# telin0411/multimodal_sequencing

Hardware: AMD Instinct MI355X
Metric: multimodal steps/sec (fwd+bwd) at N=5 steps, seq=512, ViT-B/16; 1/2/4/8 GPU (higher is better)
Workload: dtype bf16; 1 GPU; config3: ViT-B/16 + 12x768 joint encoder + BERSON, N=5 steps, 20 pairs/story, pair seq 120+393=513; global_batch=32, stories_per_gpu=32, micro_batch=32, seq_len=513, parallelism=dp1

## Files before the change

multimodal_sequencing_amd/_native.py:

```python
import ctypes
import math
import os
import re

import torch

_HERE = os.path.dirname(os.path.abspath(__file__))
LIB_PATH = os.path.join(_HERE, "_lib", "libmmseq.so")
HEADER_PATH = os.path.join(os.path.dirname(_HERE), "include", "mmseq.h")

_vp = ctypes.c_void_p


class Rows(ctypes.Structure):
    _fields_ = [("ld", ctypes.c_int64), ("bstride", ctypes.c_int64), ("rpb", ctypes.c_int64)]


def rows(ld, bstride=0, rpb=1 << 62):
    return Rows(ld, bstride, rpb)


class Dropout(ctypes.Structure):
    _fields_ = [("p", ctypes.c_float), ("stream", ctypes.c_uint32), ("seed", ctypes.c_uint64)]

# ... 52 lines not shown
               for body, name in take(r"typedef\s+struct\s*\{([^}]*)\}\s*(\w+)\s*;")}
    sigs = {}
    for decl in filter(None, (d.strip() for d in text.split(";"))):
        if decl == "}":
            continue
        m = re.fullmatch(r"(mmseq_status|int64_t|const\s+char\s*\*)\s*(mmseq_\w+)\s*\(([^()]*)\)", decl)
        if not m:
            raise NativeError(f"mmseq.h: cannot parse declaration {' '.join(decl.split())!r}")
        args = [] if m[3].strip() in ("", "void") else m[3].split(",")
        sigs[m[2]] = (_RETURNS[re.sub(r"\s*\*", "*", " ".join(m[1].split()))],
                      [(_dp if re.search(r"\bmmseq_dropout\b", a) else _vp) if "*" in a
                       else scalar(a, m[2]) for a in args])
    return sigs, consts, structs


def _read_header():
    if not os.path.exists(HEADER_PATH):
        raise NativeError(f"mmseq C header not found at {HEADER_PATH}; the binding reads every "
                          "signature and constant from it.")
    with open(HEADER_PATH) as f:
        return f.read()


_SIGS, CONSTANTS, STRUCTS = parse_header(_read_header())

F32, BF16 = CONSTANTS["MMSEQ_F32"], CONSTANTS["MMSEQ_BF16"]
ACT = {"none": CONSTANTS["MMSEQ_ACT_NONE"], "gelu": CONSTANTS["MMSEQ_ACT_GELU_ERF"],
       "quickgelu": CONSTANTS["MMSEQ_ACT_QUICKGELU"], "tanh": CONSTANTS["MMSEQ_ACT_TANH"],
       "gelu_tanh": CONSTANTS["MMSEQ_ACT_GELU_TANH"]}
EUNSUPPORTED = CONSTANTS["MMSEQ_EUNSUPPORTED"]
XENT_EVAL_MAX_K = CONSTANTS["MMSEQ_XENT_EVAL_MAX_K"]

WORKSPACE_BYTES = 256 << 20
_ws = {}


def gemm_workspace(device, stream=None):
    dev = torch.device(device)
    if stream is None:
        stream = torch.cuda.current_stream(dev)
    key = (dev.index if dev.index is not None else torch.cuda.current_device(), stream.cuda_stream)
    buf = _ws.get(key)
    if buf is None:
        buf = _ws[key] = torch.empty(WORKSPACE_BYTES // 4, dtype=torch.float32, device=dev)
    return buf


GEMM_AUTO = CONSTANTS["MMSEQ_GEMM_AUTO"]
_sel = {"gemm": GEMM_AUTO, "attn": 1}
_lib = None


def lib():
    global _lib
    if _lib is None:
        if not os.path.exists(LIB_PATH):
            raise NativeError(
                f"mmseq HIP library not found at {LIB_PATH}; run __graft_entry__.build() "
                "(make -C multimodal_sequencing_amd/csrc). There is no CPU fallback.")
        L = ctypes.CDLL(LIB_PATH)
        for name, (res, args) in _SIGS.items():
            fn = getattr(L, name)
            fn.restype = res
            fn.argtypes = args
        _lib = L
    return _lib


def _check(st, what):
    if st != 0:
        raise NativeError(f"{what} failed ({st}): {lib().mmseq_last_error().decode()}")


def _status(st, name):
    if st != EUNSUPPORTED:
        _check(st, name)
# ... 123 lines not shown


def attn_fwd_rows(P, T, Tq, heads, qkv, key_bias, scale, out, lse, drop=None, keep_bits=None):
    _dev(qkv, out, lse)
    H = heads * 64
    _call("mmseq_attn_fwd_rows", P, T, Tq, heads, _p(qkv), 3 * H, 0, H, 2 * H, _p(key_bias), scale,
          _p(out), H, _p(lse), _d(drop), _p(keep_bits))


def attn_bwd_rows(P, T, Tq, heads, qkv, key_bias, scale, out, dout, lse, delta, dqkv, drop=None,
                  keep_bits=None):
    _dev(qkv, out, dout, dqkv)
    H = heads * 64
    _call("mmseq_attn_bwd_rows", P, T, Tq, heads, _p(qkv), 3 * H, 0, H, 2 * H, _p(key_bias), scale,
          _p(out), H, _p(dout), H, _p(lse), _p(delta), _p(dqkv), 3 * H, _d(drop), _p(keep_bits))


def small_attn_fwd(B, T, heads, d, q, k, v, key_bias, scale, out, probs, drop=None):
    _call("mmseq_small_attn_fwd", B, T, heads, d, _p(q), _p(k), _p(v), _p(key_bias), scale, _p(out),
          _p(probs), _d(drop))


def small_attn_bwd(B, T, heads, d, q, k, v, probs, dout, scale, dq, dk, dv, drop=None):
    _call("mmseq_small_attn_bwd", B, T, heads, d, _p(q), _p(k), _p(v), _p(probs), _p(dout), scale,
          _p(dq), _p(dk), _p(dv), _d(drop))


def layernorm_fwd(nrows, cols, x, xl, gamma, beta, eps, y, yl, mean, rstd, drop=None):
    _dev(x, y, gamma, beta)
    _call("mmseq_layernorm_fwd", nrows, cols, _p(x), xl, _p(gamma), _p(beta), eps, _p(y), yl,
# ... 626 lines not shown
```

multimodal_sequencing_amd/csrc/attention.hip:

```cpp
#include "gemm_common.h"
#include "launch_plan.h"
#include <type_traits>

namespace {

using namespace mmseq_plan;

constexpr int HD = 64;
constexpr int QT = 64;
constexpr float NEG = -1e30f;

template <typename TI> struct ACfg;
template <> struct ACfg<unsigned short> { static constexpr int LD = 80, VE = 8; };
template <> struct ACfg<float> { static constexpr int LD = 68, VE = 4; };

template <typename TI> struct V16;
template <> struct V16<unsigned short> { typedef u16x8 T; };
template <> struct V16<float> { typedef f32x4 T; };

struct AttnArgs {
  int P, T, heads;
  const void* qkv; int64_t ld_qkv, q_off, k_off, v_off;
  const float* key_bias; float scale;
  const void* out; int64_t ld_out;
  const void* dout; int64_t ld_dout;
  float* lse; float* delta;
  void* dqkv; int64_t ld_dqkv;
  void* o_w;
  Drop drop;
  uint64_t* bits;
  int nkt2;
  int tail0, nxq, xoff, nxl;
  int Tq;
  uint8_t* q8; int64_t ldq8; uint8_t* q8s;
};

template <typename TI>
__device__ __forceinline__ void stage_tile(TI* s, const TI* base, int64_t ld, int r0, int T,
                                           int tid) {
  typedef typename V16<TI>::T V;
  constexpr int VE = ACfg<TI>::VE, LD = ACfg<TI>::LD;
  constexpr int CPR = HD / VE;
  constexpr int NCH = (QT * CPR) / 256;
#pragma unroll
  for (int c = 0; c < NCH; ++c) {
    int L = c * 256 + tid;
    int r = L / CPR, cc = L % CPR;
    V v;
    if (r0 + r < T) {
// ... 1333 lines not shown
      unsigned short* op = reinterpret_cast<unsigned short*>(a.o_w) + ((int64_t)p * T + q) * a.ld_out +
                           h * 64 + 4 * hh;
#pragma unroll
      for (int db = 0; db < 2; ++db)
#pragma unroll
        for (int jj = 0; jj < 4; ++jj) {
          const f32x4 v = {o[qb][db][4 * jj], o[qb][db][4 * jj + 1], o[qb][db][4 * jj + 2],
                           o[qb][db][4 * jj + 3]};
          Vec4<unsigned short>::st(op + db * 32 + 8 * jj, v * inv);
        }
      if (hh == 0) a.lse[((int64_t)p * a.heads + h) * T + q] = (m[qb] + __builtin_amdgcn_logf(lt)) * LN2;
    }
  }
}

template <int DMODE>
__global__ __launch_bounds__(256, DMODE == 0 ? 4 : 2) void attn_dq_bf16_kernel(AttnArgs a) {
  constexpr bool DROP = DMODE != 0;
  extern __shared__ __attribute__((aligned(16))) unsigned short smem[];
  float* sBias = reinterpret_cast<float*>(smem + 4 * IMG);
  const int tid = threadIdx.x, lane = tid & 63;
  const int wave = __builtin_amdgcn_readfirstlane(tid >> 6);
  const int g = lane >> 4, i = lane & 15;
  const int T = a.T;
  const BlkIdx bi = attn_block((a.Tq + 127) >> 7, a.heads);
  const int h = bi.h, p = bi.p;
  const int nkt = (T + 63) >> 6;
  const int qw = bi.x * 128 + wave * 32;
  const bool active = qw < a.Tq;
  const int64_t ld = a.ld_qkv;
  const rsrc_t rk = head_rsrc(a.qkv, (int64_t)p * T, ld, a.k_off + h * 64, T);
  const rsrc_t rv = head_rsrc(a.qkv, (int64_t)p * T, ld, a.v_off + h * 64, T);
  const uint32_t loff = dma_lane_off(lane, ld);
  const rsrc_t rbits = DMODE == 2 ? make_rsrc(a.bits + ((int64_t)p * a.heads + h) * T * a.nkt2,
                                              (int64_t)T * a.nkt2 * 8)
                                  : make_rsrc(a.qkv, 0);
  const uint32_t boff0 = (uint32_t)(((qw + i) * a.nkt2 * 4 + g) * 2);
  auto stage = [&](int t) {
    unsigned short* kimg = smem + (t & 1) * 2 * IMG;
#pragma unroll
// ... 41 lines not shown
    for (int ks = 0; ks < 2; ++ks) {
      const u16x8 x = __builtin_bit_cast(u16x8, of[grp][ks]), y = __builtin_bit_cast(u16x8, ovf[grp][ks]);
#pragma unroll
      for (int e = 0; e < 8; ++e) dot = fmaf(bf2f(x[e]), bf2f(y[e]), dot);
    }
    dot += __shfl_xor(dot, 16, 64);
    dot += __shfl_xor(dot, 32, 64);
    Dd[grp] = dot;
    const int64_t ri = ((int64_t)p * a.heads + h) * T + q;
    L2[grp] = q < a.Tq ? L2[grp] * LOG2E : 1e30f;
    if (q < a.Tq && g == 0) a.delta[ri] = dot;
    settle(qf[grp][0]);
    settle(qf[grp][1]);
    settle(L2[grp]);
  }
  const float c = a.scale * LOG2E;
  const int Tp4 = (T + 3) & ~3;
  uint64_t drow[2];
#pragma unroll
  for (int grp = 0; grp < 2; ++grp)
    drow[grp] = (((uint64_t)p * a.heads + h) * T + (qw + grp * 16 + i)) * Tp4;
  constexpr bool DQ_LINIT = DMODE == 2;
  f32x4 linit[2];
#pragma unroll
  for (int grp = 0; grp < 2; ++grp) {
    const float nl = -L2[grp] / c;
    linit[grp] = (f32x4){nl, nl, nl, nl};
  }
  f32x4 dq[2][4];
#pragma unroll
// ... 73 lines not shown
      }
      dsf[grp][0] = pack_pair(dp[grp][0], dp[grp][1]);
      dsf[grp][1] = pack_pair(dp[grp][2], dp[grp][3]);
    }
#pragma unroll
    for (int d = 0; d < 4; ++d) {
      const bf16x8_t k0 = lds_tr(kimg, to[d]), k1 = lds_tr(kimg, 32 * 64 + to[d]);
#pragma unroll
      for (int grp = 0; grp < 2; ++grp) {
        dq[grp][d] = mma(k0, dsf[grp][0], dq[grp][d]);
        dq[grp][d] = mma(k1, dsf[grp][1], dq[grp][d]);
      }
    }
  }
  asm volatile("s_waitcnt vmcnt(0)" ::: "memory");
  if (!active) return;
#pragma unroll
  for (int grp = 0; grp < 2; ++grp) {
    const int q = qw + grp * 16 + i;
    if (q < T) {
      unsigned short* dqp = reinterpret_cast<unsigned short*>(a.dqkv) +
                            ((int64_t)p * T + q) * a.ld_dqkv + a.q_off + h * 64 + 4 * g;
#pragma unroll
      for (int d = 0; d < 4; ++d) Vec4<unsigned short>::st(dqp + d * 16, dq[grp][d] * a.scale);
      if (a.q8) q8_head_row(a, (int64_t)p * T + q, (int)a.q_off + h * 64, dq[grp], a.scale, g);
    }
  }
}

__device__ __forceinline__ void zero_dq(const AttnArgs& a, unsigned short* row, int h, int g) {
  unsigned short* dqp = row + a.q_off + h * 64 + 4 * g;
#pragma unroll
  for (int d = 0; d < 4; ++d) Vec4<unsigned short>::st(dqp + d * 16, (f32x4){0.f, 0.f, 0.f, 0.f});
}

template <int DMODE, bool FOLD>
__global__ __launch_bounds__(256, FOLD || DMODE == 1 ? 2 : 3) void attn_dkdv_bf16_kernel(AttnArgs a) {
  constexpr bool DROP = DMODE != 0;
  extern __shared__ __attribute__((aligned(16))) unsigned short smem[];
  const int T = a.T, Tq = a.Tq;
  const int nqt = (Tq + 63) >> 6;
  float* sL = reinterpret_cast<float*>(smem + 4 * IMG);
  float* sD = sL + nqt * 64;
  unsigned short* sBits = reinterpret_cast<unsigned short*>(sD + nqt * 64);
  unsigned short* sBitsT = sBits + 1024;
  u16x8* sKVt = reinterpret_cast<u16x8*>(sBitsT + 1024);
  const int tid = threadIdx.x, lane = tid & 63;
  const int wave = __builtin_amdgcn_readfirstlane(tid >> 6);
  const int g = lane >> 4, i = lane & 15;
  BlkIdx bi = attn_block(a.nxl, a.heads);
  bi.x += a.xoff;
// ... 271 lines not shown
        unsigned short* dkp = row + a.k_off + h * 64 + 4 * g;
        unsigned short* dvp = row + a.v_off + h * 64 + 4 * g;
#pragma unroll
        for (int d = 0; d < 4; ++d) {
          Vec4<unsigned short>::st(dkp + d * 16, dkt[d] * a.scale);
          Vec4<unsigned short>::st(dvp + d * 16, dvt[d]);
        }
        if (a.q8) {
          q8_head_row(a, (int64_t)p * T + key, (int)a.k_off + h * 64, dkt, a.scale, g);
          q8_head_row(a, (int64_t)p * T + key, (int)a.v_off + h * 64, dvt, 1.f, g);
        }
        if (key >= Tq) zero_dq(a, row, h, g);
      }
    }
  }
  if (!active) return;
#pragma unroll
  for (int grp = 0; grp < 2; ++grp) {
    const int key = kw + grp * 16 + i;
    if (key < T) {
      unsigned short* row = reinterpret_cast<unsigned short*>(a.dqkv) + ((int64_t)p * T + key) * a.ld_dqkv;
      unsigned short* dkp = row + a.k_off + h * 64 + 4 * g;
      unsigned short* dvp = row + a.v_off + h * 64 + 4 * g;
#pragma unroll
      for (int d = 0; d < 4; ++d) {
        Vec4<unsigned short>::st(dkp + d * 16, dk[grp][d] * a.scale);
        Vec4<unsigned short>::st(dvp + d * 16, dv[grp][d]);
      }
      if (a.q8) {
        q8_head_row(a, (int64_t)p * T + key, (int)a.k_off + h * 64, dk[grp], a.scale, g);
        q8_head_row(a, (int64_t)p * T + key, (int)a.v_off + h * 64, dv[grp], 1.f, g);
      }
      if (key >= Tq) zero_dq(a, row, h, g);
    }
  }
}

bool aligned16(const void* p) { return ((uintptr_t)p & 15) == 0; }

mmseq_status check_common(int P, int T, int heads, const void* qkv, int64_t ld, int64_t qo,
                          int64_t ko, int64_t vo, mmseq_dtype dt) {
  MMSEQ_REQUIRE(P >= 0 && T > 0 && heads > 0, "attn: bad sizes P=%d T=%d heads=%d", P, T, heads);
  MMSEQ_REQUIRE(dt == MMSEQ_F32 || dt == MMSEQ_BF16, "attn: bad dtype");
  const int ve = dt == MMSEQ_BF16 ? 8 : 4;
  MMSEQ_REQUIRE(aligned16(qkv) && ld % ve == 0 && qo % ve == 0 && ko % ve == 0 && vo % ve == 0,
                "attn: qkv must be 16-byte aligned with ld/offsets multiple of %d", ve);
  MMSEQ_REQUIRE(qo + heads * 64 <= ld && ko + heads * 64 <= ld && vo + heads * 64 <= ld,
                "attn: head slices exceed the row");
  return MMSEQ_OK;
// ... 14 lines not shown
typedef void (*AttnKernel)(AttnArgs);
typedef const AttnKernel FwdFamily[3][2];
FwdFamily FWD32 = {{attn_fwd32_kernel<0, false>, attn_fwd32_kernel<0, false>},
                   {attn_fwd32_kernel<1, false>, attn_fwd32_kernel<1, true>},
                   {attn_fwd32_kernel<2, false>, attn_fwd32_kernel<2, true>}};
FwdFamily FWD16 = {{attn_fwd_bf16_kernel<0, false>, attn_fwd_bf16_kernel<0, false>},
                   {attn_fwd_bf16_kernel<1, false>, attn_fwd_bf16_kernel<1, true>},
                   {attn_fwd_bf16_kernel<2, false>, attn_fwd_bf16_kernel<2, true>}};
FwdFamily FWD16_Q8 = {{attn_fwd_bf16_kernel<0, false, true>, attn_fwd_bf16_kernel<0, false, true>},
                      {attn_fwd_bf16_kernel<1, false, true>, attn_fwd_bf16_kernel<1, true, true>},
                      {attn_fwd_bf16_kernel<2, false, true>, attn_fwd_bf16_kernel<2, true, true>}};
const AttnKernel DQ16[3] = {attn_dq_bf16_kernel<0>, attn_dq_bf16_kernel<1>, attn_dq_bf16_kernel<2>};
const AttnKernel DKDV16[3][2] = {{attn_dkdv_bf16_kernel<0, false>, attn_dkdv_bf16_kernel<0, true>},
                                 {attn_dkdv_bf16_kernel<1, false>, nullptr},
                                 {attn_dkdv_bf16_kernel<2, false>, attn_dkdv_bf16_kernel<2, true>}};

void launch_fwd(FwdFamily& k, const AttnFwdPlan& p, const AttnArgs& a, hipStream_t s) {
  hipLaunchKernelGGL(k[p.dmode][p.wide], dim3(p.blocks), dim3(p.threads), (size_t)p.lds_bytes, s, a);
}

}

static mmseq_status attn_fwd_impl(int P, int T, int Tq, int heads, const void* qkv, int64_t ld_qkv,
                                  int64_t q_off, int64_t k_off, int64_t v_off,
                                  const float* key_bias, float scale, void* out, int64_t ld_out,
                                  float* lse, mmseq_dtype dtype, const mmseq_dropout* drop,
                                  uint64_t* keep_bits, int variant, mmseq_stream stream) {
  mmseq_status st = check_common(P, T, heads, qkv, ld_qkv, q_off, k_off, v_off, dtype);
  if (st) return st;
  MMSEQ_REQUIRE(out && lse && ld_out >= heads * 64, "attn_fwd: bad out/lse");
// ... 30 lines not shown
                                            int64_t v_off, const float* key_bias, float scale,
                                            void* out, int64_t ld_out, float* lse,
                                            const mmseq_dropout* drop, uint64_t* keep_bits,
                                            mmseq_stream stream) {
  return attn_fwd_impl(P, T, Tq, heads, qkv, ld_qkv, q_off, k_off, v_off, key_bias, scale, out,
                       ld_out, lse, MMSEQ_BF16, drop, keep_bits, 1, stream);
}

static mmseq_status attn_bwd_impl(int P, int T, int Tq, int heads, const void* qkv, int64_t ld_qkv,
                                  int64_t q_off, int64_t k_off, int64_t v_off,
                                  const float* key_bias, float scale, const void* out,
                                  int64_t ld_out, const void* dout, int64_t ld_dout,
                                  const float* lse, float* delta, void* dqkv, int64_t ld_dqkv,
                                  mmseq_dtype dtype, const mmseq_dropout* drop,
                                  const uint64_t* keep_bits, int variant, void* q8, int64_t ldq8,
                                  void* q8_scales, mmseq_stream stream) {
  mmseq_status st = check_common(P, T, heads, qkv, ld_qkv, q_off, k_off, v_off, dtype);
  if (st) return st;
  const int ve = dtype == MMSEQ_BF16 ? 8 : 4;
  MMSEQ_REQUIRE(out && dout && lse && delta && dqkv, "attn_bwd: null buffer");
  MMSEQ_REQUIRE(aligned16(dout) && ld_dout % ve == 0, "attn_bwd: dout alignment");
  const int64_t hi_off = q_off > k_off ? (q_off > v_off ? q_off : v_off) : (k_off > v_off ? k_off : v_off);
  MMSEQ_REQUIRE(hi_off + (int64_t)heads * 64 <= ld_dqkv,
                "attn_bwd: head slices exceed the dqkv row (ld_dqkv=%lld)", (long long)ld_dqkv);
  MMSEQ_REQUIRE(Tq >= 1 && Tq <= T && (Tq == T || (dtype == MMSEQ_BF16 && variant && !q8)),
                "attn_bwd: Tq=%d (1 <= Tq <= T; Tq < T needs the bf16 fast kernels, no MX-fp8 copy)", Tq);
  if (P == 0) return MMSEQ_OK;
  AttnArgs a = attn_args(P, T, Tq, heads, qkv, ld_qkv, q_off, k_off, v_off, key_bias, scale, drop, keep_bits);
  a.out = out; a.ld_out = ld_out; a.dout = dout; a.ld_dout = ld_dout;
  a.lse = const_cast<float*>(lse); a.delta = delta; a.dqkv = dqkv; a.ld_dqkv = ld_dqkv;
  a.q8 = reinterpret_cast<uint8_t*>(q8); a.ldq8 = ldq8; a.q8s = reinterpret_cast<uint8_t*>(q8_scales);
  if (q8 && !(dtype == MMSEQ_BF16 && variant))
    return mmseq_set_error(MMSEQ_EUNSUPPORTED, "attn_bwd_mxfp8: the bf16 fast kernels only");
  hipStream_t s = reinterpret_cast<hipStream_t>(stream);
  const int64_t rows = (int64_t)P * T;
  dim3 gd((unsigned)((rows + 3) / 4));
  dim3 grid((T + QT - 1) / QT, heads, P);
  if (dtype == MMSEQ_BF16 && variant) {
    MMSEQ_REQUIRE(aligned16(out) && ld_out % 8 == 0 && aligned16(dqkv) && ld_dqkv % 8 == 0,
                  "attn_bwd: out / dqkv must be 16-byte aligned rows");
    const AttnBwdPlan bp = attn_bwd_plan(P, T, Tq, heads, a.drop.thr != 0, keep_bits != nullptr);
    hipLaunchKernelGGL(DQ16[bp.dmode], dim3(bp.dq_blocks), dim3(256), (size_t)bp.dq_lds, s, a);
    AttnArgs ak = a;
    ak.tail0 = bp.tail0; ak.nxq = bp.nxq;
    ak.xoff = 0; ak.nxl = bp.nplain;
    if (bp.nplain)
      hipLaunchKernelGGL(DKDV16[bp.dmode][0], dim3(bp.plain_blocks), dim3(256), (size_t)bp.dkdv_lds, s, ak);
    ak.xoff = bp.nplain; ak.nxl = 1;
    if (bp.ntail)
      hipLaunchKernelGGL(DKDV16[bp.dmode][1], dim3(bp.tail_blocks), dim3(256), (size_t)bp.tail_lds, s, ak);
  } else if (dtype == MMSEQ_BF16) {
    hipLaunchKernelGGL(attn_delta_kernel<unsigned short>, gd, dim3(256), 0, s, a);
    hipLaunchKernelGGL(attn_dkdv_kernel<unsigned short>, grid, dim3(256), 0, s, a);
    hipLaunchKernelGGL(attn_dq_kernel<unsigned short>, grid, dim3(256), 0, s, a);
  } else {
// ... 2 lines not shown
    hipLaunchKernelGGL(attn_dq_kernel<float>, grid, dim3(256), 0, s, a);
  }
  return mmseq_check_launch("attn_bwd");
}

extern "C" mmseq_status mmseq_attn_bwd(int P, int T, int heads, const void* qkv, int64_t ld_qkv,
                                       int64_t q_off, int64_t k_off, int64_t v_off,
                                       const float* key_bias, float scale, const void* out,
                                       int64_t ld_out, const void* dout, int64_t ld_dout,
                                       const float* lse, float* delta, void* dqkv,
                                       int64_t ld_dqkv, mmseq_dtype dtype,
                                       const mmseq_dropout* drop, const uint64_t* keep_bits,
                                       int variant, mmseq_stream stream) {
  return attn_bwd_impl(P, T, T, heads, qkv, ld_qkv, q_off, k_off, v_off, key_bias, scale, out, ld_out,
                       dout, ld_dout, lse, delta, dqkv, ld_dqkv, dtype, drop, keep_bits, variant,
                       nullptr, 0, nullptr, stream);
}

extern "C" mmseq_status mmseq_attn_bwd_rows(int P, int T, int Tq, int heads, const void* qkv,
                                            int64_t ld_qkv, int64_t q_off, int64_t k_off,
                                            int64_t v_off, const float* key_bias, float scale,
                                            const void* out, int64_t ld_out, const void* dout,
                                            int64_t ld_dout, const float* lse, float* delta,
                                            void* dqkv, int64_t ld_dqkv, const mmseq_dropout* drop,
                                            const uint64_t* keep_bits, mmseq_stream stream) {
  return attn_bwd_impl(P, T, Tq, heads, qkv, ld_qkv, q_off, k_off, v_off, key_bias, scale, out, ld_out,
                       dout, ld_dout, lse, delta, dqkv, ld_dqkv, MMSEQ_BF16, drop, keep_bits, 1,
                       nullptr, 0, nullptr, stream);
}

extern "C" mmseq_status mmseq_attn_bwd_mxfp8(int P, int T, int heads, const void* qkv,
                                             int64_t ld_qkv, const float* key_bias, float scale,
                                             const void* out, int64_t ld_out, const void* dout,
                                             int64_t ld_dout, const float* lse, float* delta,
                                             void* dqkv, int64_t ld_dqkv,
                                             const mmseq_dropout* drop, const uint64_t* keep_bits,
                                             void* q8, int64_t ldq8, void* q8_scales,
                                             mmseq_stream stream) {
  const int64_t H = (int64_t)heads * 64;
  MMSEQ_REQUIRE(q8 && q8_scales && ldq8 >= 3 * H && ldq8 % 16 == 0 && ((uintptr_t)q8 & 15) == 0,
                "attn_bwd_mxfp8: q8 / ldq8");
  return attn_bwd_impl(P, T, T, heads, qkv, ld_qkv, 0, H, 2 * H, key_bias, scale, out, ld_out, dout,
                       ld_dout, lse, delta, dqkv, ld_dqkv, MMSEQ_BF16, drop, keep_bits, 1, q8, ldq8,
                       q8_scales, stream);
}

extern "C" int64_t mmseq_attn_keep_bits_words(int P, int T, int heads) {
  return keep_bits_words(P, T, heads);
}

extern "C" mmseq_status mmseq_attn_fwd_mxfp8_dual(int P, int T, int heads, const void* qkv,
                                                  int64_t ld_qkv, int64_t q_off, int64_t k_off,
                                                  int64_t v_off, const float* key_bias, float scale,
                                                  void* out, int64_t ld_out, float* lse,
                                                  const mmseq_dropout* drop, uint64_t* keep_bits,
                                                  void* q8, int64_t ldq8, void* q8_scales,
                                                  mmseq_stream stream) {
  mmseq_status st = check_common(P, T, heads, qkv, ld_qkv, q_off, k_off, v_off, MMSEQ_BF16);
  if (st) return st;
// ... 23 lines not shown
```

multimodal_sequencing_amd/csrc/launch_plan.h:

```cpp
#pragma once
#include <cstdint>

namespace mmseq_plan {

inline int64_t ceil_div(int64_t a, int64_t b) { return (a + b - 1) / b; }

constexpr int RCH = 64;

inline int reduce_rows(int nb) { return (int)ceil_div(nb, RCH); }
inline int64_t reduce_extra(int nb, int W) { return (int64_t)reduce_rows(nb) * W; }
inline int64_t partials_floats(int nb, int W) { return (int64_t)nb * W + reduce_extra(nb, W); }

constexpr int CS_ROWS = 256;

struct ColsumPlan {
  int nb;
  int64_t red_off;
  int64_t floats;
};

inline ColsumPlan colsum_plan(int rows, int cols) {
  const int nb = (int)ceil_div(rows, CS_ROWS);
  return {nb, (int64_t)nb * cols, partials_floats(nb, cols)};
}
// ... 142 lines not shown
  p.dmode = dropout ? (keep_bits ? 2 : 1) : 0;
  p.nkt2 = attn_nkt2(T);
  p.dq_blocks = attn_blocks((Tq + 127) / 128, heads, P);
  p.dq_lds = ATTN_KV_LDS + (int64_t)attn_nkt(T) * 64 * 4;
  const TailFold f = tail_fold(T, p.dmode != 1);
  p.tail0 = f.tail0; p.nxq = f.nxq;
  p.ntail = f.tail0 ? 1 : 0;
  p.nplain = f.nxq - p.ntail;
  p.plain_blocks = attn_blocks(p.nplain, heads, P);
  p.tail_blocks = attn_blocks(p.ntail, heads, P);
  p.dkdv_lds = ATTN_KV_LDS + (int64_t)attn_nkt(T) * 64 * 4 * 2 + 2048;
  p.tail_lds = p.dkdv_lds + 6144;
  return p;
}

}
```

multimodal_sequencing_amd/kernels.py:

```python
import math
import os

import torch

from . import _native as N

GELU, QGELU, TANH, GELU_TANH = (N.ACT[a] for a in ("gelu", "quickgelu", "tanh", "gelu_tanh"))


def _rows(ld):
    return N.rows(ld)


def _colsum(x, out):
    rows = x.numel() // x.shape[-1]
    N.colsum(x, rows, x.shape[-1], x.shape[-1], out, accumulate=True)


def _wgrad(dy, x, gW, gb=None):
    N.gemm_wgrad(dy, x, gW, gb)


def _linear(x, W, bias=None, act=0, aux=None, resid=None, out=None, out_dtype=None, drop=None):
    R = x.numel() // x.shape[-1]
# ... 154 lines not shown
                                                 dx_drop=dx_drop, drop_dx=drop_dx)), dsum
        N.layernorm_bwd(R, C, dy, _rows(C), x, _rows(C), mean, rstd, gamma, dx,
                        dx_rows if dx_rows is not None else _rows(C), dres, _rows(C), dgamma, dbeta,
                        dx_drop=dx_drop, drop_dx=drop_dx,
                        dx_drop_rows=dx_drop_rows, dsum=dsum, dsum_with_dres=dsum_with_dres)
        return _Act(g), None

    def attn_bwd(self, P, T, heads, qkv, key_bias, o, do, lse, drop=None, keep_bits=None, Tq=None):
        H = qkv.shape[-1] // 3
        scale = 1.0 / math.sqrt(H // heads)
        dqkv = torch.empty_like(qkv)
        delta = torch.empty(P, heads, T, device=qkv.device)
        if self.f8dg:
            return _Act(dqkv, N.attn_bwd_mxfp8(P, T, heads, qkv, key_bias, scale, o, do, lse, delta, dqkv,
                                               drop=drop, keep_bits=keep_bits))
        if Tq is not None and Tq < T:
            N.attn_bwd_rows(P, T, Tq, heads, qkv, key_bias, scale, o, do, lse, delta, dqkv, drop=drop,
                            keep_bits=keep_bits)
        else:
            N.attn_bwd(P, T, heads, qkv, 3 * H, 0, H, 2 * H, key_bias, scale, o, H, do, H, lse, delta,
                       dqkv, 3 * H, drop=drop, keep_bits=keep_bits)
        return _Act(dqkv)

    def bwd_done(self):
        _fp8_bwd_done(self.f8dg)


def _engine(kind, st, x, Ws, save, drops=(None, None, None), Tq=None):
    plain = _Engine(st, save=save)
    if not _FP8["on"] or x.dtype != torch.bfloat16 or Tq is not None:
        return plain
# ... 837 lines not shown
```

Before: 2.637 steps/s.

## Handle short attention tails in backward via cross-emitting kernels and finish pass

When the sequence length is a multiple of 128 plus 1-16 rows (e.g. 513), the dQ and dK/dV backward kernels now emit partial tail contributions into a workspace. A small finish kernel then combines them instead of processing a mostly empty extra 128-row block. The dQ kernel also computes delta for the tail rows. This adds a workspace allocation per call, a third kernel launch, and extra LDS reductions in exchange for dropping padded tail-block work.

New measurement: 2.654 steps/s, median of 6. Within noise of the previous version (+0.7%).

```diff
diff --git a/include/mmseq_attn_tails.h b/include/mmseq_attn_tails.h
--- /dev/null
+++ b/include/mmseq_attn_tails.h
@@ -0,0 +1,20 @@
+#ifndef MMSEQ_ATTN_TAILS_H
+#define MMSEQ_ATTN_TAILS_H
+#include "mmseq.h"
+
+#ifdef __cplusplus
+extern "C" {
+#endif
+
+int64_t mmseq_attn_bwd_workspace_size(int P, int T, int Tq, int heads);
+mmseq_status mmseq_attn_bwd_ws(int P, int T, int Tq, int heads, const void* qkv, int64_t ld_qkv,
+                               int64_t q_off, int64_t k_off, int64_t v_off, const float* key_bias,
+                               float scale, const void* out, int64_t ld_out, const void* dout,
+                               int64_t ld_dout, const float* lse, float* delta, void* dqkv,
+                               int64_t ld_dqkv, const mmseq_dropout* drop,
+                               const uint64_t* keep_bits, void* workspace, int64_t workspace_bytes,
+                               mmseq_stream stream);
+#ifdef __cplusplus
+}
+#endif
+#endif
diff --git a/multimodal_sequencing_amd/_native.py b/multimodal_sequencing_amd/_native.py
--- a/multimodal_sequencing_amd/_native.py
+++ b/multimodal_sequencing_amd/_native.py
@@ -8,6 +8,7 @@
 _HERE = os.path.dirname(os.path.abspath(__file__))
 LIB_PATH = os.path.join(_HERE, "_lib", "libmmseq.so")
 HEADER_PATH = os.path.join(os.path.dirname(_HERE), "include", "mmseq.h")
+EXT_HEADER_PATH = os.path.join(os.path.dirname(_HERE), "include", "mmseq_attn_tails.h")
 
 _vp = ctypes.c_void_p
 
@@ -90,15 +91,17 @@
     return sigs, consts, structs
 
 
-def _read_header():
-    if not os.path.exists(HEADER_PATH):
-        raise NativeError(f"mmseq C header not found at {HEADER_PATH}; the binding reads every "
+def _read_header(path=None):
+    path = HEADER_PATH if path is None else path
+    if not os.path.exists(path):
+        raise NativeError(f"mmseq C header not found at {path}; the binding reads every "
                           "signature and constant from it.")
-    with open(HEADER_PATH) as f:
+    with open(path) as f:
         return f.read()
 
 
 _SIGS, CONSTANTS, STRUCTS = parse_header(_read_header())
+_EXT_SIGS = parse_header(_read_header(EXT_HEADER_PATH))[0]
 
 F32, BF16 = CONSTANTS["MMSEQ_F32"], CONSTANTS["MMSEQ_BF16"]
 ACT = {"none": CONSTANTS["MMSEQ_ACT_NONE"], "gelu": CONSTANTS["MMSEQ_ACT_GELU_ERF"],
@@ -123,7 +126,7 @@
 
 
 GEMM_AUTO = CONSTANTS["MMSEQ_GEMM_AUTO"]
-_sel = {"gemm": GEMM_AUTO, "attn": 1}
+_sel = {"gemm": GEMM_AUTO, "attn": 1, "attn_tails": 1}
 _lib = None
 
 
@@ -135,7 +138,7 @@
                 f"mmseq HIP library not found at {LIB_PATH}; run __graft_entry__.build() "
                 "(make -C multimodal_sequencing_amd/csrc). There is no CPU fallback.")
         L = ctypes.CDLL(LIB_PATH)
-        for name, (res, args) in _SIGS.items():
+        for name, (res, args) in list(_SIGS.items()) + list(_EXT_SIGS.items()):
             fn = getattr(L, name)
             fn.restype = res
             fn.argtypes = args
@@ -289,6 +292,23 @@
     H = heads * 64
     _call("mmseq_attn_bwd_rows", P, T, Tq, heads, _p(qkv), 3 * H, 0, H, 2 * H, _p(key_bias), scale,
           _p(out), H, _p(dout), H, _p(lse), _p(delta), _p(dqkv), 3 * H, _d(drop), _p(keep_bits))
+
+
+def attn_tails_set(mode):
+    _sel["attn_tails"] = int(mode)
+
+
+def attn_bwd_workspace(P, T, Tq, heads):
+    return lib().mmseq_attn_bwd_workspace_size(P, T, Tq, heads)
+
+
+def attn_bwd_ws(P, T, Tq, heads, qkv, key_bias, scale, out, dout, lse, delta, dqkv, ws, drop=None,
+                keep_bits=None):
+    _dev(qkv, out, dout, dqkv, ws)
+    H = heads * 64
+    _call("mmseq_attn_bwd_ws", P, T, Tq, heads, _p(qkv), 3 * H, 0, H, 2 * H, _p(key_bias), scale,
+          _p(out), H, _p(dout), H, _p(lse), _p(delta), _p(dqkv), 3 * H, _d(drop), _p(keep_bits),
+          _p(ws), 0 if ws is None else ws.numel() * ws.element_size())
 
 
 def small_attn_fwd(B, T, heads, d, q, k, v, key_bias, scale, out, probs, drop=None):
diff --git a/multimodal_sequencing_amd/csrc/attention.hip b/multimodal_sequencing_amd/csrc/attention.hip
--- a/multimodal_sequencing_amd/csrc/attention.hip
+++ b/multimodal_sequencing_amd/csrc/attention.hip
@@ -1,5 +1,7 @@
 #include "gemm_common.h"
 #include "launch_plan.h"
+#include "attn_tail_plan.h"
+#include "../../include/mmseq_attn_tails.h"
 #include <type_traits>
 
 namespace {
@@ -33,6 +35,7 @@
   int tail0, nxq, xoff, nxl;
   int Tq;
   uint8_t* q8; int64_t ldq8; uint8_t* q8s;
+  float* ws; AttnTailPlan tp;
 };
 
 template <typename TI>
@@ -1396,8 +1399,44 @@
   }
 }
 
-template <int DMODE>
-__global__ __launch_bounds__(256, DMODE == 0 ? 4 : 2) void attn_dq_bf16_kernel(AttnArgs a) {
+__device__ __forceinline__ void tail_stage(unsigned short* xw, const bf16x8_t (&f)[2][2], int lane) {
+  asm volatile("s_waitcnt lgkmcnt(0)" ::: "memory");
+#pragma unroll
+  for (int grp = 0; grp < 2; ++grp)
+#pragma unroll
+    for (int ks = 0; ks < 2; ++ks)
+      *reinterpret_cast<u16x8*>(xw + grp * 1024 + row_off(lane, ks)) = __builtin_bit_cast(u16x8, f[grp][ks]);
+  asm volatile("s_waitcnt lgkmcnt(0)" ::: "memory");
+}
+__device__ __forceinline__ void tail_product(const unsigned short* xw, const unsigned short* w, int lane,
+                                             f32x4 (&acc)[4]) {
+  typedef __attribute__((ext_vector_type(4))) unsigned short u16x4;
+  const int g = lane >> 4, i = lane & 15;
+  const u16x4 lo = *reinterpret_cast<const u16x4*>(w + i * 32 + 4 * g);
+  const u16x4 hi = *reinterpret_cast<const u16x4*>(w + i * 32 + 16 + 4 * g);
+  const u16x8 b = {lo[0], lo[1], lo[2], lo[3], hi[0], hi[1], hi[2], hi[3]};
+  const bf16x8_t bf = __builtin_bit_cast(bf16x8_t, b);
+#pragma unroll
+  for (int d = 0; d < 4; ++d) acc[d] = mma(lds_tr(xw, tr_off(lane, d)), bf, (f32x4){0.f, 0.f, 0.f, 0.f});
+}
+__device__ __forceinline__ void tail_reduce_put(float* red, int wave, int lane, const f32x4 (&acc)[4]) {
+#pragma unroll
+  for (int d = 0; d < 4; ++d)
+#pragma unroll
+    for (int r = 0; r < 4; ++r) red[(wave * 16 + d * 4 + r) * 64 + lane] = acc[d][r];
+}
+__device__ __forceinline__ void tail_reduce_store(const float* red, int wave, int lane, float* out, int rows) {
+  const int g = lane >> 4, i = lane & 15;
+  f32x4 v = (f32x4){0.f, 0.f, 0.f, 0.f};
+#pragma unroll
+  for (int w = 0; w < 4; ++w)
+#pragma unroll
+    for (int r = 0; r < 4; ++r) v[r] += red[(w * 16 + wave * 4 + r) * 64 + lane];
+  if (i < rows) *reinterpret_cast<f32x4*>(out + i * 64 + wave * 16 + 4 * g) = v;
+}
+
+template <int DMODE, bool EMIT = false>
+__global__ __launch_bounds__(256, DMODE == 0 ? 4 : (EMIT ? 3 : 2)) void attn_dq_bf16_kernel(AttnArgs a) {
   constexpr bool DROP = DMODE != 0;
   extern __shared__ __attribute__((aligned(16))) unsigned short smem[];
   float* sBias = reinterpret_cast<float*>(smem + 4 * IMG);
@@ -1405,7 +1444,7 @@
   const int wave = __builtin_amdgcn_readfirstlane(tid >> 6);
   const int g = lane >> 4, i = lane & 15;
   const int T = a.T;
-  const BlkIdx bi = attn_block((a.Tq + 127) >> 7, a.heads);
+  const BlkIdx bi = attn_block(EMIT ? a.tp.nqb : (a.Tq + 127) >> 7, a.heads);
   const int h = bi.h, p = bi.p;
   const int nkt = (T + 63) >> 6;
   const int qw = bi.x * 128 + wave * 32;
@@ -1477,6 +1516,22 @@
     settle(qf[grp][1]);
     settle(L2[grp]);
   }
+  if (EMIT && a.tp.nkb > 0 && bi.x == a.tp.nqb - 1) {
+    typedef unsigned int u32x2b __attribute__((ext_vector_type(2)));
+    const int q = a.tp.tail0 + (tid >> 4);
+    const uint32_t co = (uint32_t)(tid & 15) * 8u;
+    const u32x2b x = __builtin_amdgcn_raw_buffer_load_b64(rdo, (uint32_t)((int64_t)q * a.ld_dout * 2) + co, 0, 0);
+    const u32x2b y = __builtin_amdgcn_raw_buffer_load_b64(rout, (uint32_t)((int64_t)q * a.ld_out * 2) + co, 0, 0);
+    float dot = 0.f;
+#pragma unroll
+    for (int e = 0; e < 2; ++e) {
+      dot = fmaf(bf2f((unsigned short)(x[e] & 0xFFFFu)), bf2f((unsigned short)(y[e] & 0xFFFFu)), dot);
+      dot = fmaf(bf2f((unsigned short)(x[e] >> 16)), bf2f((unsigned short)(y[e] >> 16)), dot);
+    }
+#pragma unroll
+    for (int sh = 1; sh < 16; sh <<= 1) dot += __shfl_xor(dot, sh, 64);
+    if ((tid & 15) == 0 && q < a.Tq) a.delta[((int64_t)p * a.heads + h) * T + q] = dot;
+  }
   const float c = a.scale * LOG2E;
   const int Tp4 = (T + 3) & ~3;
   uint64_t drow[2];
@@ -1580,11 +1635,11 @@
     }
   }
   asm volatile("s_waitcnt vmcnt(0)" ::: "memory");
-  if (!active) return;
+  if (!EMIT && !active) return;
 #pragma unroll
   for (int grp = 0; grp < 2; ++grp) {
     const int q = qw + grp * 16 + i;
-    if (q < T) {
+    if (active && q < T) {
       unsigned short* dqp = reinterpret_cast<unsigned short*>(a.dqkv) +
                             ((int64_t)p * T + q) * a.ld_dqkv + a.q_off + h * 64 + 4 * g;
 #pragma unroll
@@ -1592,6 +1647,67 @@
       if (a.q8) q8_head_row(a, (int64_t)p * T + q, (int)a.q_off + h * 64, dq[grp], a.scale, g);
     }
   }
+  if constexpr (EMIT) {
+    uint32_t lnu;
+    asm volatile("v_mbcnt_lo_u32_b32 %0, -1, 0\n\tv_mbcnt_hi_u32_b32 %0, -1, %0" : "=v"(lnu));
+    const int ln = (int)lnu, g = ln >> 4, i = ln & 15;
+    f32x4 ptl[2], dstl[2];
+#pragma unroll
+    for (int grp = 0; grp < 2; ++grp) ptl[grp] = dstl[grp] = (f32x4){0.f, 0.f, 0.f, 0.f};
+    if (active) {
+      const int t = nkt - 1;
+      const unsigned short* kimg = smem + (t & 1) * 2 * IMG;
+      const unsigned short* vimg = kimg + IMG;
+      const int ro0 = row_off(ln, 0), ro1 = row_off(ln, 1);
+      const bf16x8_t k0 = lds_row(kimg, ro0), k1 = lds_row(kimg, ro1);
+      const bf16x8_t v0 = lds_row(vimg, ro0), v1 = lds_row(vimg, ro1);
+      const f32x4 bias = *reinterpret_cast<const f32x4*>(sBias + t * 64 + 4 * g);
+      const uint32_t scale_u = __float_as_uint(a.drop.scale);
+#pragma unroll
+      for (int grp = 0; grp < 2; ++grp) {
+        uint32_t kw16 = 0xFFFFu;
+        if (DMODE == 2)
+          kw16 = reinterpret_cast<const unsigned short*>(a.bits)[
+              ((((int64_t)p * a.heads + h) * T + qw + grp * 16 + i) * a.nkt2 + t) * 4 + g];
+        f32x4 sc = mma(k0, qf[grp][0], DQ_LINIT ? linit[grp] : (f32x4){0.f, 0.f, 0.f, 0.f});
+        sc = mma(k1, qf[grp][1], sc);
+        f32x4 dpt = mma(v0, of[grp][0], (f32x4){0.f, 0.f, 0.f, 0.f});
+        dpt = mma(v1, of[grp][1], dpt);
+#pragma unroll
+        for (int r = 0; r < 4; ++r) {
+          float dm = 1.f;
+          if (DMODE == 2) dm = __uint_as_float((uint32_t)__builtin_amdgcn_sbfe((int)kw16, r, 1) & scale_u);
+          const float pv = DQ_LINIT ? ex2(fmaf(sc[r], c, bias[r])) : ex2(fmaf(sc[r], c, bias[r]) - L2[grp]);
+          ptl[grp][r] = DROP ? pv * dm : pv;
+          dstl[grp][r] = pv * fmaf(dpt[r], dm, -Dd[grp]);
+        }
+      }
+    }
+    __syncthreads();
+    unsigned short* xw = smem + wave * 2048;
+    unsigned short* ww = smem + 8192 + wave * 1024;
+    float* redv = reinterpret_cast<float*>(smem);
+    float* redk = reinterpret_cast<float*>(smem + 8192);
+#pragma unroll
+    for (int grp = 0; grp < 2; ++grp)
+#pragma unroll
+      for (int r = 0; r < 4; ++r) {
+        ww[(4 * g + r) * 32 + grp * 16 + i] = f2bf(ptl[grp][r]);
+        ww[512 + (4 * g + r) * 32 + grp * 16 + i] = f2bf(dstl[grp][r]);
+      }
+    f32x4 av[4], ak[4];
+    tail_stage(xw, of, ln);
+    tail_product(xw, ww, ln, av);
+    tail_stage(xw, qf, ln);
+    tail_product(xw, ww + 512, ln, ak);
+    __syncthreads();
+    tail_reduce_put(redv, wave, ln, av);
+    tail_reduce_put(redk, wave, ln, ak);
+    __syncthreads();
+    const int64_t bh = (int64_t)p * a.heads + h;
+    tail_reduce_store(redv, wave, ln, a.ws + tail_dv_slot(a.tp, bh, bi.x), a.tp.tail);
+    tail_reduce_store(redk, wave, ln, a.ws + tail_dk_slot(a.tp, bh, bi.x), a.tp.tail);
+  }
 }
 
 __device__ __forceinline__ void zero_dq(const AttnArgs& a, unsigned short* row, int h, int g) {
@@ -1600,7 +1716,7 @@
   for (int d = 0; d < 4; ++d) Vec4<unsigned short>::st(dqp + d * 16, (f32x4){0.f, 0.f, 0.f, 0.f});
 }
 
-template <int DMODE, bool FOLD>
+template <int DMODE, bool FOLD, bool EMIT = false>
 __global__ __launch_bounds__(256, FOLD || DMODE == 1 ? 2 : 3) void attn_dkdv_bf16_kernel(AttnArgs a) {
   constexpr bool DROP = DMODE != 0;
   extern __shared__ __attribute__((aligned(16))) unsigned short smem[];
@@ -1902,7 +2018,58 @@
       }
     }
   }
-  if (!active) return;
+  if (!EMIT && !active) return;
+  if constexpr (EMIT) {
+    uint32_t lnu;
+    asm volatile("v_mbcnt_lo_u32_b32 %0, -1, 0\n\tv_mbcnt_hi_u32_b32 %0, -1, %0" : "=v"(lnu));
+    const int ln = (int)lnu, g = ln >> 4, i = ln & 15;
+    static_assert(!FOLD && DMODE != 1, "the cross-emitting dK/dV kernel: plain blocks, LINIT modes");
+    f32x4 dst[2];
+    {
+      const int t = nqt - 1;
+      const unsigned short* qimg = smem + (t & 1) * 2 * IMG;
+      const unsigned short* oimg = qimg + IMG;
+      const int ro0 = row_off(ln, 0), ro1 = row_off(ln, 1);
+      const bf16x8_t q0 = lds_row(qimg, ro0), q1 = lds_row(qimg, ro1);
+      const bf16x8_t o0 = lds_row(oimg, ro0), o1 = lds_row(oimg, ro1);
+      const f32x4 lrow = *reinterpret_cast<const f32x4*>(sL + t * 64 + 4 * g);
+      const f32x4 Dq = *reinterpret_cast<const f32x4*>(sD + t * 64 + 4 * g);
+      const uint32_t scale_u = __float_as_uint(a.drop.scale);
+      const uint32_t* bw = reinterpret_cast<const uint32_t*>(sBits + (t & 1) * 512) +
+                           (wave >> 1) * 2 + ((i >> 3) & 1);
+      const uint32_t pos0 = ((i >> 2) & 1) * 16 + (wave & 1) * 8 + (i & 3);
+#pragma unroll
+      for (int grp = 0; grp < 2; ++grp) {
+        f32x4 sc = mma(q0, kf[grp][0], lrow);
+        sc = mma(q1, kf[grp][1], sc);
+        f32x4 dpt = mma(o0, vf[grp][0], (f32x4){0.f, 0.f, 0.f, 0.f});
+        dpt = mma(o1, vf[grp][1], dpt);
+#pragma unroll
+        for (int r = 0; r < 4; ++r) {
+          const float pv = ex2(fmaf(sc[r], c, kb2[grp]));
+          float mk = 1.f;
+          if (DMODE == 2)
+            mk = __uint_as_float((uint32_t)__builtin_amdgcn_sbfe((int)bw[(4 * g + r) * 4], pos0 + 4 * grp, 1) & scale_u);
+          dst[grp][r] = pv * (DROP ? fmaf(dpt[r], mk, Dq[r]) : dpt[r] + Dq[r]);
+        }
+      }
+    }
+    __syncthreads();
+    unsigned short* xw = smem + wave * 2048;
+    unsigned short* ww = smem + 8192 + wave * 512;
+    float* red = reinterpret_cast<float*>(smem);
+#pragma unroll
+    for (int grp = 0; grp < 2; ++grp)
+#pragma unroll
+      for (int r = 0; r < 4; ++r) ww[(4 * g + r) * 32 + grp * 16 + i] = f2bf(dst[grp][r]);
+    f32x4 aq[4];
+    tail_stage(xw, kf, ln);
+    tail_product(xw, ww, ln, aq);
+    asm volatile("s_waitcnt lgkmcnt(0)" ::: "memory");
+    tail_reduce_put(red, wave, ln, aq);
+    __syncthreads();
+    tail_reduce_store(red, wave, ln, a.ws + tail_dq_slot(a.tp, (int64_t)p * a.heads + h, bi.x), a.tp.tail);
+  }
 #pragma unroll
   for (int grp = 0; grp < 2; ++grp) {
     const int key = kw + grp * 16 + i;
@@ -1921,6 +2088,83 @@
       }
       if (key >= Tq) zero_dq(a, row, h, g);
     }
+  }
+}
+
+template <int DMODE>
+__global__ __launch_bounds__(256) void attn_tail_finish_kernel(AttnArgs a) {
+  extern __shared__ __attribute__((aligned(16))) unsigned short fsm[];
+  constexpr int FS = TAIL_FINISH_FS;
+  const int tid = threadIdx.x, lane = tid & 63, w = tid >> 6;
+  const int64_t bh = blockIdx.x;
+  const int p = (int)(bh / a.heads), h = (int)(bh % a.heads);
+  const int T = a.T, n = a.tp.tail, t0 = a.tp.tail0;
+  const bool rowsq = a.tp.nkb > 0;
+  unsigned short *sQ = fsm, *sK = sQ + n * FS, *sV = sK + n * FS, *sO = sV + n * FS;
+  float* sP = reinterpret_cast<float*>(sO + n * FS);
+  float* sS = sP + n * 16;
+  const unsigned short* qkv = reinterpret_cast<const unsigned short*>(a.qkv) + ((int64_t)p * T + t0) * a.ld_qkv + h * 64 + lane;
+  const unsigned short* dob = reinterpret_cast<const unsigned short*>(a.dout) + ((int64_t)p * a.Tq + t0) * a.ld_dout + h * 64 + lane;
+  for (int r = w; r < n; r += 4) {
+    sK[r * FS + lane] = qkv[r * a.ld_qkv + a.k_off];
+    sV[r * FS + lane] = qkv[r * a.ld_qkv + a.v_off];
+    sQ[r * FS + lane] = rowsq ? qkv[r * a.ld_qkv + a.q_off] : (unsigned short)0;
+    sO[r * FS + lane] = rowsq ? dob[r * a.ld_dout] : (unsigned short)0;
+  }
+  __syncthreads();
+  {
+    const int r = tid >> 4, k = tid & 15;
+    if (r < n) {
+      float pv = 0.f, ds = 0.f;
+      if (rowsq && k < n) {
+        float s = 0.f, dp = 0.f;
+#pragma unroll 2
+        for (int d8 = 0; d8 < 8; ++d8) {
+          const u16x8 q8 = *reinterpret_cast<const u16x8*>(sQ + r * FS + d8 * 8);
+          const u16x8 k8 = *reinterpret_cast<const u16x8*>(sK + k * FS + d8 * 8);
+          const u16x8 o8 = *reinterpret_cast<const u16x8*>(sO + r * FS + d8 * 8);
+          const u16x8 v8 = *reinterpret_cast<const u16x8*>(sV + k * FS + d8 * 8);
+#pragma unroll
+          for (int e = 0; e < 8; ++e) {
+            s = fmaf(bf2f(q8[e]), bf2f(k8[e]), s);
+            dp = fmaf(bf2f(o8[e]), bf2f(v8[e]), dp);
+          }
+        }
+        const float c = a.scale * LOG2E;
+        const float kb = a.key_bias ? a.key_bias[(int64_t)p * T + t0 + k] * LOG2E : 0.f;
+        const float L = a.lse[bh * T + t0 + r] * LOG2E, D = a.delta[bh * T + t0 + r];
+        const float pe = ex2(fmaf(s, c, kb) - L);
+        float mk = 1.f;
+        if (DMODE == 2) {
+          const uint64_t wd = a.bits[(bh * T + t0 + r) * a.nkt2 + (t0 >> 6)];
+          mk = ((wd >> (((k >> 2) & 3) * 16 + (k & 3))) & 1) ? a.drop.scale : 0.f;
+        }
+        pv = pe * mk;
+        ds = pe * fmaf(dp, mk, -D);
+      }
+      sP[r * 16 + k] = pv;
+      sS[r * 16 + k] = ds;
+    }
+  }
+  __syncthreads();
+  unsigned short* out = reinterpret_cast<unsigned short*>(a.dqkv) + ((int64_t)p * T + t0) * a.ld_dqkv + h * 64 + lane;
+  for (int r = w; r < n; r += 4) {
+    float dq = 0.f, dv = 0.f, dk = 0.f;
+    for (int kb = 0; kb < a.tp.nkb; ++kb) dq += a.ws[tail_dq_slot(a.tp, bh, kb) + r * 64 + lane];
+    for (int qb = 0; qb < a.tp.nqb; ++qb) {
+      dv += a.ws[tail_dv_slot(a.tp, bh, qb) + r * 64 + lane];
+      dk += a.ws[tail_dk_slot(a.tp, bh, qb) + r * 64 + lane];
+    }
+    if (rowsq) {
+      for (int k = 0; k < n; ++k) {
+        dq = fmaf(sS[r * 16 + k], bf2f(sK[k * FS + lane]), dq);
+        dv = fmaf(sP[k * 16 + r], bf2f(sO[k * FS + lane]), dv);
+        dk = fmaf(sS[k * 16 + r], bf2f(sQ[k * FS + lane]), dk);
+      }
+    }
+    out[r * a.ld_dqkv + a.q_off] = f2bf(dq * a.scale);
+    out[r * a.ld_dqkv + a.k_off] = f2bf(dk * a.scale);
+    out[r * a.ld_dqkv + a.v_off] = f2bf(dv);
   }
 }
 
@@ -1965,6 +2209,10 @@
 const AttnKernel DKDV16[3][2] = {{attn_dkdv_bf16_kernel<0, false>, attn_dkdv_bf16_kernel<0, true>},
                                  {attn_dkdv_bf16_kernel<1, false>, nullptr},
                                  {attn_dkdv_bf16_kernel<2, false>, attn_dkdv_bf16_kernel<2, true>}};
+const AttnKernel DQ16_EMIT[3] = {attn_dq_bf16_kernel<0, true>, nullptr, attn_dq_bf16_kernel<2, true>};
+const AttnKernel DKDV16_EMIT[3] = {attn_dkdv_bf16_kernel<0, false, true>, nullptr,
+                                   attn_dkdv_bf16_kernel<2, false, true>};
+const AttnKernel TAIL_FINISH[3] = {attn_tail_finish_kernel<0>, nullptr, attn_tail_finish_kernel<2>};
 
 void launch_fwd(FwdFamily& k, const AttnFwdPlan& p, const AttnArgs& a, hipStream_t s) {
   hipLaunchKernelGGL(k[p.dmode][p.wide], dim3(p.blocks), dim3(p.threads), (size_t)p.lds_bytes, s, a);
@@ -2025,7 +2273,7 @@
                                   const float* lse, float* delta, void* dqkv, int64_t ld_dqkv,
                                   mmseq_dtype dtype, const mmseq_dropout* drop,
                                   const uint64_t* keep_bits, int variant, void* q8, int64_t ldq8,
-                                  void* q8_scales, mmseq_stream stream) {
+                                  void* q8_scales, void* ws, int64_t ws_bytes, mmseq_stream stream) {
   mmseq_status st = check_common(P, T, heads, qkv, ld_qkv, q_off, k_off, v_off, dtype);
   if (st) return st;
   const int ve = dtype == MMSEQ_BF16 ? 8 : 4;
@@ -2050,6 +2298,17 @@
   if (dtype == MMSEQ_BF16 && variant) {
     MMSEQ_REQUIRE(aligned16(out) && ld_out % 8 == 0 && aligned16(dqkv) && ld_dqkv % 8 == 0,
                   "attn_bwd: out / dqkv must be 16-byte aligned rows");
+    const AttnBwdTailPlan tl = attn_bwd_tail_plan(P, T, Tq, heads, a.drop.thr != 0, keep_bits != nullptr);
+    if (tl.on && !q8 && ws && aligned16(ws) && ws_bytes >= tl.ws_bytes) {
+      a.ws = reinterpret_cast<float*>(ws);
+      a.tp = attn_tail_plan(P, T, Tq, heads);
+      a.xoff = 0; a.nxl = tl.nkb;
+      hipLaunchKernelGGL(DQ16_EMIT[tl.dmode], dim3(tl.dq_blocks), dim3(256), (size_t)tl.dq_lds, s, a);
+      hipLaunchKernelGGL(tl.emit_dq ? DKDV16_EMIT[tl.dmode] : DKDV16[tl.dmode][0], dim3(tl.dkdv_blocks),
+                         dim3(256), (size_t)tl.dkdv_lds, s, a);
+      hipLaunchKernelGGL(TAIL_FINISH[tl.dmode], dim3(tl.finish_blocks), dim3(256), (size_t)tl.finish_lds, s, a);
+      return mmseq_check_launch("attn_bwd");
+    }
     const AttnBwdPlan bp = attn_bwd_plan(P, T, Tq, heads, a.drop.thr != 0, keep_bits != nullptr);
     hipLaunchKernelGGL(DQ16[bp.dmode], dim3(bp.dq_blocks), dim3(256), (size_t)bp.dq_lds, s, a);
     AttnArgs ak = a;
@@ -2082,7 +2341,7 @@
                                        int variant, mmseq_stream stream) {
   return attn_bwd_impl(P, T, T, heads, qkv, ld_qkv, q_off, k_off, v_off, key_bias, scale, out, ld_out,
                        dout, ld_dout, lse, delta, dqkv, ld_dqkv, dtype, drop, keep_bits, variant,
-                       nullptr, 0, nullptr, stream);
+                       nullptr, 0, nullptr, nullptr, 0, stream);
 }
 
 extern "C" mmseq_status mmseq_attn_bwd_rows(int P, int T, int Tq, int heads, const void* qkv,
@@ -2094,7 +2353,7 @@
                                             const uint64_t* keep_bits, mmseq_stream stream) {
   return attn_bwd_impl(P, T, Tq, heads, qkv, ld_qkv, q_off, k_off, v_off, key_bias, scale, out, ld_out,
                        dout, ld_dout, lse, delta, dqkv, ld_dqkv, MMSEQ_BF16, drop, keep_bits, 1,
-                       nullptr, 0, nullptr, stream);
+                       nullptr, 0, nullptr, nullptr, 0, stream);
 }
 
 extern "C" mmseq_status mmseq_attn_bwd_mxfp8(int P, int T, int heads, const void* qkv,
@@ -2110,7 +2369,24 @@
                 "attn_bwd_mxfp8: q8 / ldq8");
   return attn_bwd_impl(P, T, T, heads, qkv, ld_qkv, 0, H, 2 * H, key_bias, scale, out, ld_out, dout,
                        ld_dout, lse, delta, dqkv, ld_dqkv, MMSEQ_BF16, drop, keep_bits, 1, q8, ldq8,
-                       q8_scales, stream);
+                       q8_scales, nullptr, 0, stream);
+}
+
+extern "C" int64_t mmseq_attn_bwd_workspace_size(int P, int T, int Tq, int heads) {
+  return attn_tail_plan(P, T, Tq, heads).bytes;
+}
+
+extern "C" mmseq_status mmseq_attn_bwd_ws(int P, int T, int Tq, int heads, const void* qkv,
+                                          int64_t ld_qkv, int64_t q_off, int64_t k_off, int64_t v_off,
+                                          const float* key_bias, float scale, const void* out,
+                                          int64_t ld_out, const void* dout, int64_t ld_dout,
+                                          const float* lse, float* delta, void* dqkv, int64_t ld_dqkv,
+                                          const mmseq_dropout* drop, const uint64_t* keep_bits,
+                                          void* workspace, int64_t workspace_bytes,
+                                          mmseq_stream stream) {
+  return attn_bwd_impl(P, T, Tq, heads, qkv, ld_qkv, q_off, k_off, v_off, key_bias, scale, out, ld_out,
+                       dout, ld_dout, lse, delta, dqkv, ld_dqkv, MMSEQ_BF16, drop, keep_bits, 1,
+                       nullptr, 0, nullptr, workspace, workspace_bytes, stream);
 }
 
 extern "C" int64_t mmseq_attn_keep_bits_words(int P, int T, int heads) {
diff --git a/multimodal_sequencing_amd/csrc/attn_tail_plan.h b/multimodal_sequencing_amd/csrc/attn_tail_plan.h
--- /dev/null
+++ b/multimodal_sequencing_amd/csrc/attn_tail_plan.h
@@ -0,0 +1,44 @@
+#pragma once
+#include <cstdint>
+
+#if defined(__HIPCC__)
+#define MMSEQ_TAIL_HD __host__ __device__
+#else
+#define MMSEQ_TAIL_HD
+#endif
+
+namespace mmseq_plan {
+
+struct AttnTailPlan {
+  int tail0;
+  int tail;
+  int nkb;
+  int nqb;
+  int64_t per_bh;
+  int64_t bytes;
+};
+
+MMSEQ_TAIL_HD inline AttnTailPlan attn_tail_plan(int P, int T, int Tq, int heads) {
+  AttnTailPlan p = {0, 0, 0, 0, 0, 0};
+  const int n = T / 128, r = T % 128;
+  if (n < 1 || r < 1 || r > 16 || Tq < 1 || (Tq != T && Tq > n * 128)) return p;
+  p.tail0 = n * 128;
+  p.tail = r;
+  p.nkb = Tq == T ? n : 0;
+  p.nqb = Tq == T ? n : (Tq + 127) / 128;
+  p.per_bh = (int64_t)(p.nkb + 2 * p.nqb) * r * 64;
+  p.bytes = (int64_t)P * heads * p.per_bh * 4;
+  return p;
+}
+
+MMSEQ_TAIL_HD inline int64_t tail_dq_slot(const AttnTailPlan& p, int64_t bh, int kb) {
+  return bh * p.per_bh + (int64_t)kb * p.tail * 64;
+}
+MMSEQ_TAIL_HD inline int64_t tail_dv_slot(const AttnTailPlan& p, int64_t bh, int qb) {
+  return bh * p.per_bh + (int64_t)(p.nkb + 2 * qb) * p.tail * 64;
+}
+MMSEQ_TAIL_HD inline int64_t tail_dk_slot(const AttnTailPlan& p, int64_t bh, int qb) {
+  return tail_dv_slot(p, bh, qb) + (int64_t)p.tail * 64;
+}
+
+}
diff --git a/multimodal_sequencing_amd/csrc/launch_plan.h b/multimodal_sequencing_amd/csrc/launch_plan.h
--- a/multimodal_sequencing_amd/csrc/launch_plan.h
+++ b/multimodal_sequencing_amd/csrc/launch_plan.h
@@ -1,5 +1,7 @@
 #pragma once
 #include <cstdint>
+
+#include "attn_tail_plan.h"
 
 namespace mmseq_plan {
 
@@ -180,4 +182,36 @@
   return p;
 }
 
-}
+struct AttnBwdTailPlan {
+  bool on;
+  int dmode, nkb, nqb;
+  bool emit_dq;
+  unsigned dq_blocks, dkdv_blocks, finish_blocks;
+  int64_t dq_lds, dkdv_lds, finish_lds;
+  int64_t ws_bytes;
+};
+
+constexpr int TAIL_FINISH_FS = 72;
+inline int64_t attn_tail_finish_lds(int tail) { return (int64_t)tail * (4 * TAIL_FINISH_FS * 2 + 2 * 16 * 4); }
+
+inline AttnBwdTailPlan attn_bwd_tail_plan(int P, int T, int Tq, int heads, bool dropout, bool keep_bits) {
+  AttnBwdTailPlan p = {};
+  p.dmode = dropout ? (keep_bits ? 2 : 1) : 0;
+  const AttnTailPlan tp = attn_tail_plan(P, T, Tq, heads);
+  p.on = p.dmode != 1 && tp.tail0 > 0;
+  if (!p.on) return p;
+  p.emit_dq = tp.nkb > 0;
+  p.nkb = tp.tail0 / 128;
+  p.nqb = tp.nqb;
+  p.dq_blocks = attn_blocks(p.nqb, heads, P);
+  p.dkdv_blocks = attn_blocks(p.nkb, heads, P);
+  p.finish_blocks = attn_blocks(1, heads, P);
+  const AttnBwdPlan b = attn_bwd_plan(P, T, Tq, heads, dropout, keep_bits);
+  p.dq_lds = b.dq_lds;
+  p.dkdv_lds = b.dkdv_lds;
+  p.finish_lds = attn_tail_finish_lds(tp.tail);
+  p.ws_bytes = tp.bytes;
+  return p;
+}
+
+}
diff --git a/multimodal_sequencing_amd/kernels.py b/multimodal_sequencing_amd/kernels.py
--- a/multimodal_sequencing_amd/kernels.py
+++ b/multimodal_sequencing_amd/kernels.py
@@ -192,7 +192,14 @@
         if self.f8dg:
             return _Act(dqkv, N.attn_bwd_mxfp8(P, T, heads, qkv, key_bias, scale, o, do, lse, delta, dqkv,
                                                drop=drop, keep_bits=keep_bits))
-        if Tq is not None and Tq < T:
+        tq = T if Tq is None else Tq
+        nws = N.attn_bwd_workspace(P, T, tq, heads) if T > 128 and 1 <= T % 128 <= 16 and \
+            N._sel["attn_tails"] and N._sel["attn"] and qkv.dtype == torch.bfloat16 else 0
+        if nws:
+            ws = torch.empty(nws // 4, device=qkv.device)
+            N.attn_bwd_ws(P, T, tq, heads, qkv, key_bias, scale, o, do, lse, delta, dqkv, ws, drop=drop,
+                          keep_bits=keep_bits)
+        elif tq < T:
             N.attn_bwd_rows(P, T, Tq, heads, qkv, key_bias, scale, o, do, lse, delta, dqkv, drop=drop,
                             keep_bits=keep_bits)
         else:
```
